# mightypirate1/DRL-Tetris

Hardware: AMD Instinct MI355X
Metric: env-steps/sec at 64k parallel 20x10 boards (higher is better)
Workload: dtype u32

## Files before the change

drl-tetris_amd/csrc/tetris_engine.h:

```cpp
#pragma once
#include "tetris_layout.h"
#include "tetris_tables.h"

#if defined(__clang__)
#define TE_UNROLL _Pragma("unroll")
#else
#define TE_UNROLL _Pragma("GCC unroll 8")
#endif

namespace te {

TE_HD int ctz32(uint32_t v) { return __builtin_ctz(v); }
TE_HD int clz32(uint32_t v) { return __builtin_clz(v); }
#if defined(__HIP_DEVICE_COMPILE__)
TE_HD uint32_t ld_stream(const uint32_t* p) { return __builtin_nontemporal_load(p); }
TE_HD void st_stream(uint32_t* p, uint32_t v) { __builtin_nontemporal_store(v, p); }
#else
TE_HD uint32_t ld_stream(const uint32_t* p) { return *p; }
TE_HD void st_stream(uint32_t* p, uint32_t v) { *p = v; }
#endif

#if defined(TE_PATH_COUNTERS) && !defined(__HIPCC__)
enum PathCounter { PC_KICK = 0, PC_KICK_2ND, PC_KICK_3RD, PC_KICK_FAILED, PC_KICK_DOWN, PC_DROP_EXACT, PC_RT_OFF_SPAWN,
                   PC_GARBAGE_ROW, PC_GARBAGE_LIFT2, PC_DEATH_GARBAGE, PC_DEATH_SPAWN, PC_TIMER_LOCK, PC_KEY_KICK, PC_KEY_KICK_FAILED,
                   PC_UNDO_SIMPLE, PC_UNDO_FULL, PC_UNDO_MISPREDICT, PC_NCOUNTERS };
extern unsigned long long te_path_count[PC_NCOUNTERS];
#define TE_COUNT(i) (te_path_count[i]++)
#else
#define TE_COUNT(i) do {} while (0)
#endif

enum MemMode : int { MEM_STREAM = 0, MEM_AGENT = 1, MEM_AFFINE = 2 };
#if defined(__HIP_DEVICE_COMPILE__)
TE_HD uint32_t ld_agent(const uint32_t* p) { return __hip_atomic_load(p, __ATOMIC_RELAXED, __HIP_MEMORY_SCOPE_AGENT); }
TE_HD void st_agent(uint32_t* p, uint32_t v) { __hip_atomic_store(p, v, __ATOMIC_RELAXED, __HIP_MEMORY_SCOPE_AGENT); }
#else
TE_HD uint32_t ld_agent(const uint32_t* p) { return *p; }
TE_HD void st_agent(uint32_t* p, uint32_t v) { *p = v; }
#endif
#if defined(__HIP_DEVICE_COMPILE__)
TE_HD __amdgpu_buffer_rsrc_t te_rsrc(const void* base) {
// ... 96 lines not shown
    const uint64_t* start;
    const double* combo_pow;
    uint32_t n_draws;
    uint32_t margin;
    int H;
    uint32_t floor_bits;
    bool tint;
    bool queue;
};

constexpr int ERR_FIFO = 1;
constexpr int ERR_STREAM = 2;

struct Raw8 { uint32_t lo, hi; };
struct Player {
    uint32_t col[NCOL];
    uint32_t tint[3][NCOL];
    int kind, rot, x, y, next;
    int dead, lock_armed, reward;
    int inc_count, combo_count, line_count, qlen;
    int q_overflow;
    int32_t time_ms, drop_delay, drop_time, speedup_time, lock_time;
    int32_t combo_start, combo_time, min_remaining;
    uint32_t combo_remaining;
    float incoming;
    uint32_t piece_draws, hole_draws;
    uint32_t pgroup;
    uint32_t lines_sent, lines_cleared, lines_blocked, max_combo, lines_seen, garbage_cleared;
    int32_t qcount[FIFO_CAP];
    int32_t qdelay[FIFO_CAP];
    int q_loaded;
    Raw8 pf_raw;
    int pf_ok;
};

struct ResetPrefetch { uint32_t seed16; uint64_t word; int ok; };

template <int P>
struct Game {
    Player pl[P];
    uint32_t seed16;
    int round_over, last_winner;
    uint32_t flags;
    uint32_t episode;
    uint32_t steps;
    uint32_t add_lines, add_sent;
    uint32_t status;
    uint32_t draw0, draw1;
};

template <class ROWS>
TE_HD void load_player_rows(const uint32_t* s, uint32_t o, const ROWS& rows, Player& q, bool tint, bool queue = true, int mem = MEM_STREAM,
                            bool errs = true) {
    for (int c = 0; c < NCOL; c++) q.col[c] = ldw_b(s, o, row_bytes(rows, W_COL0 + c), mem);
    if (tint)
        for (int k = 0; k < 3; k++)
            for (int c = 0; c < NCOL; c++) q.tint[k][c] = ldw_b(s, o, row_bytes(rows, W_TINT0 + 10 * k + c), mem);
    uint32_t w = ldw_b(s, o, row_bytes(rows, W_PIECE), mem);
    q.kind = w & 7; q.rot = (w >> 3) & 3; q.x = (int)((w >> 5) & 15) - 4; q.y = (w >> 9) & 31;
    q.next = (w >> 14) & 7; q.dead = (w >> 17) & 1; q.lock_armed = (w >> 18) & 1; q.reward = (w >> 19) & 255;
    w = ldw_b(s, o, row_bytes(rows, W_MISC), mem);
    q.inc_count = w & 255; q.combo_count = (w >> 8) & 255; q.line_count = (w >> 16) & 255;
    q.qlen = (w >> 24) & 15; q.q_overflow = (w >> 28) & 3;
    if (!queue) { q.inc_count = 0; q.qlen = 0; }
    if (!queue && !errs) q.q_overflow = 0;
    q.time_ms = (int32_t)ldw_b(s, o, row_bytes(rows, W_TIME), mem);
    w = ldw_b(s, o, row_bytes(rows, W_DROPCOMBO), mem);
    q.drop_delay = w & 0xFFFF; q.combo_remaining = w >> 16;
    q.drop_time = (int32_t)ldw_b(s, o, row_bytes(rows, W_DROP_TIME), mem);
    q.speedup_time = (int32_t)ldw_b(s, o, row_bytes(rows, W_SPEEDUP_TIME), mem);
    q.lock_time = (int32_t)ldw_b(s, o, row_bytes(rows, W_LOCK_TIME), mem);
    q.combo_start = (int32_t)ldw_b(s, o, row_bytes(rows, W_COMBO_START), mem);
    q.combo_time = (int32_t)ldw_b(s, o, row_bytes(rows, W_COMBO_TIME), mem);
    q.incoming = queue ? u2f(ldw_b(s, o, row_bytes(rows, W_INCOMING), mem)) : 0.0f;
    q.min_remaining = queue ? (int32_t)ldw_b(s, o, row_bytes(rows, W_MIN_REMAINING), mem) : 1000;
    q.piece_draws = ldw_b(s, o, row_bytes(rows, W_PIECE_DRAWS), mem);
    q.hole_draws = queue ? ldw_b(s, o, row_bytes(rows, W_HOLE_DRAWS), mem) : 0u;
    q.pgroup = ldw_b(s, o, row_bytes(rows, W_PIECE_GROUP), mem);
    w = ldw_b(s, o, row_bytes(rows, W_STATS0), mem); q.lines_sent = w & 0xFFFF; q.lines_cleared = w >> 16;
    w = ldw_b(s, o, row_bytes(rows, W_STATS1), mem); q.lines_blocked = w & 0xFFFF; q.max_combo = w >> 16;
    w = ldw_b(s, o, row_bytes(rows, W_STATS2), mem); q.lines_seen = w & 0xFFFF; q.garbage_cleared = w >> 16;
    q.q_loaded = queue && q.qlen > 0;
    q.pf_ok = 0; q.pf_raw.lo = 0; q.pf_raw.hi = 0;
    if (queue)
        for (int i = 0; i < FIFO_CAP; i++) { q.qcount[i] = 0; q.qdelay[i] = 0; }
    if (q.q_loaded) {
        for (int i = 0; i < FIFO_CAP / 2; i++) {
            uint32_t cw = ldw_b(s, o, row_bytes(rows, W_FIFO_COUNT0 + i), mem);
            q.qcount[2 * i] = (int16_t)(cw & 0xFFFF);
            q.qcount[2 * i + 1] = (int16_t)(cw >> 16);
        }
        for (int i = 0; i < FIFO_CAP; i++) q.qdelay[i] = (int32_t)ldw_b(s, o, row_bytes(rows, W_FIFO_DELAY0 + i), mem);
    }
}

TE_HD void load_player(const uint32_t* s, uint32_t o, size_t ws, Player& q, bool tint, bool queue = true, int mem = MEM_STREAM) {
    load_player_rows(s, o, RowStride{ws}, q, tint, queue, mem);
}

template <int P, class ROWS>
TE_HD void load_game_words_rows(const Ref& gr, const ROWS& rows, Game<P>& g, bool counters = false, int mem = MEM_STREAM) {
    uint32_t meta = ldw_b(gr.s, gr.o, row_bytes(rows, G_META), mem);
    g.seed16 = meta & 0xFFFFu;
    g.round_over = (meta >> 16) & 1;
    g.last_winner = (int)((meta >> 17) & 0xF) - 1;
    g.flags = (meta >> 21) & 7u;
    g.episode = ldw_b(gr.s, gr.o, row_bytes(rows, G_EPISODE), mem);
    g.steps = counters ? ldw_b(gr.s, gr.o, row_bytes(rows, G_STEPS), mem) : 0u;
    g.add_lines = 0; g.add_sent = 0;
    g.status = 0;
}

template <int P>
TE_HD void load_game_words(const Ref& gr, Game<P>& g, bool counters = false, int mem = MEM_STREAM) {
    load_game_words_rows<P>(gr, RowStride{gr.ws}, g, counters, mem);
}
// ... 27 lines not shown
    stw_b(s, o, row_bytes(rows, W_MISC), (uint32_t)(q.inc_count & 255) | ((uint32_t)(q.combo_count & 255) << 8) |
                             ((uint32_t)(q.line_count & 255) << 16) | ((uint32_t)q.qlen << 24) | ((uint32_t)q.q_overflow << 28), mem);
    stw_b(s, o, row_bytes(rows, W_TIME), (uint32_t)q.time_ms, mem);
    stw_b(s, o, row_bytes(rows, W_DROPCOMBO), ((uint32_t)q.drop_delay & 0xFFFF) | (q.combo_remaining << 16), mem);
    stw_b(s, o, row_bytes(rows, W_DROP_TIME), (uint32_t)q.drop_time, mem);
    stw_b(s, o, row_bytes(rows, W_SPEEDUP_TIME), (uint32_t)q.speedup_time, mem);
    stw_b(s, o, row_bytes(rows, W_LOCK_TIME), (uint32_t)q.lock_time, mem);
    stw_b(s, o, row_bytes(rows, W_COMBO_START), (uint32_t)q.combo_start, mem);
    stw_b(s, o, row_bytes(rows, W_COMBO_TIME), (uint32_t)q.combo_time, mem);
    if (queue) stw_b(s, o, row_bytes(rows, W_INCOMING), f2u(q.incoming), mem);
    stw_b(s, o, row_bytes(rows, W_MIN_REMAINING), (uint32_t)q.min_remaining, mem);
    stw_b(s, o, row_bytes(rows, W_PIECE_DRAWS), q.piece_draws, mem);
    if (queue) stw_b(s, o, row_bytes(rows, W_HOLE_DRAWS), q.hole_draws, mem);
    stw_b(s, o, row_bytes(rows, W_PIECE_GROUP), q.pgroup, mem);
    stw_b(s, o, row_bytes(rows, W_STATS0), (q.lines_sent & 0xFFFF) | (q.lines_cleared << 16), mem);
    stw_b(s, o, row_bytes(rows, W_STATS1), (q.lines_blocked & 0xFFFF) | (q.max_combo << 16), mem);
    stw_b(s, o, row_bytes(rows, W_STATS2), (q.lines_seen & 0xFFFF) | (q.garbage_cleared << 16), mem);
    if (queue && (q.q_loaded || q.qlen > 0)) {
        for (int i = 0; i < FIFO_CAP / 2; i++)
            stw_b(s, o, row_bytes(rows, W_FIFO_COUNT0 + i), ((uint32_t)q.qcount[2 * i] & 0xFFFF) | ((uint32_t)q.qcount[2 * i + 1] << 16), mem);
        for (int i = 0; i < FIFO_CAP; i++) stw_b(s, o, row_bytes(rows, W_FIFO_DELAY0 + i), (uint32_t)q.qdelay[i], mem);
    }
}

TE_HD void store_player(uint32_t* s, uint32_t o, size_t ws, const Player& q, bool tint, bool queue = true, int mem = MEM_STREAM) {
    store_player_rows(s, o, RowStride{ws}, q, tint, queue, mem);
}

template <int P, class ROWS>
TE_HD void store_game_words_rows(const Ref& gr, const ROWS& rows, const Game<P>& g, bool counters = false, int mem = MEM_STREAM) {
    stw_b(gr.s, gr.o, row_bytes(rows, G_META), g.seed16 | ((uint32_t)g.round_over << 16) | ((uint32_t)(g.last_winner + 1) << 17) | (g.flags << 21), mem);
    stw_b(gr.s, gr.o, row_bytes(rows, G_EPISODE), g.episode, mem);
    if (counters) stw_b(gr.s, gr.o, row_bytes(rows, G_STEPS), g.steps, mem);
    if (g.add_lines) add_word((uint32_t*)((char*)gr.s + row_bytes(rows, G_LINES) + gr.o), g.add_lines);
    if (g.add_sent) add_word((uint32_t*)((char*)gr.s + row_bytes(rows, G_SENT) + gr.o), g.add_sent);
}

template <int P>
TE_HD void store_game_words(const Ref& gr, const Game<P>& g, bool counters = false, int mem = MEM_STREAM) {
    store_game_words_rows<P>(gr, RowStride{gr.ws}, g, counters, mem);
}

template <int P, class ROWS, class GROWS>
TE_HD void store_game_rows(const Geo& geo_in, size_t slot, const ROWS& rows, const GROWS& grows, const Game<P>& g, bool tint = false, bool queue = true,
                           bool counters = false, int mem = MEM_STREAM) {
    Geo geo = geo_in;
    geo.P = P;
    store_game_words_rows<P>(game_ref(geo, slot), grows, g, counters, mem);
    TE_UNROLL
    for (int p = 0; p < P; p++) {
        const Ref r = board_ref(geo, p, slot);
        store_player_rows(r.s, r.o, rows, g.pl[p], tint, queue, mem);
    }
}
template <int P>
TE_HD void store_game(const Geo& geo_in, size_t slot, const Game<P>& g, bool tint = false, bool queue = true, bool counters = false, int mem = MEM_STREAM) {
    store_game_rows<P>(geo_in, slot, RowStride{(size_t)P * geo_in.stride}, RowStride{geo_in.stride}, g, tint, queue, counters, mem);
}


TE_HD uint32_t shape_of(const Ctx& cx, int kind, int rot) { return cx.shapes[(kind << 2) | rot]; }

TE_HD uint64_t band_window(const Ctx& cx, const Player& q, int y) {
    uint32_t lo = 0xFFu, hi = 0xFFFF0000u;
    for (int c = 0; c < 6; c++) lo |= ((uint32_t)((int32_t)(q.col[c] | cx.floor_bits) >> y) & 0xFu) << (4 * c + 8);
    for (int c = 6; c < NCOL; c++) hi |= ((uint32_t)((int32_t)(q.col[c] | cx.floor_bits) >> y) & 0xFu) << (4 * (c - 6));
    return ((uint64_t)hi << 32) | lo;
}
// ... 54 lines not shown
    const uint32_t lo = hi2 ? (hi1 ? 0u : w2) : (hi1 ? w1 : w0);
    const uint32_t hi = hi2 ? 0u : (hi1 ? w2 : w1);
#if defined(__HIP_DEVICE_COMPILE__)
    const uint32_t under = __builtin_amdgcn_alignbyte(hi, lo, xs & 3u);
#else
    const uint32_t under = (uint32_t)((((uint64_t)hi << 32) | lo) >> (8 * (xs & 3u)));
#endif
    const uint32_t sum = under + drop_word;
    const uint32_t b0 = sum & 0xFFu, b1 = (sum >> 8) & 0xFFu, b2 = (sum >> 16) & 0xFFu, b3 = sum >> 24;
    const uint32_t m01 = b0 < b1 ? b0 : b1, m23 = b2 < b3 ? b2 : b3;
    const uint32_t m = m01 < m23 ? m01 : m23;
    if (m - 0x40u > 0x3Eu) { TE_COUNT(PC_DROP_EXACT); return drop_distance(cx, q, shape); }
    return (int)(m - 0x40u);
}

TE_HD void stamp(const Ctx& cx, Player& q, uint32_t shape) {
    unsigned xs = (unsigned)(q.x + 2);
    if (xs > 12u) return;
    uint64_t placed = (uint64_t)(shape & 0xFFFFu) << (4 * xs);
    for (int c = 0; c < NCOL; c++) {
        const uint32_t cells = ((uint32_t)(placed >> (4 * c + 8)) & 0xFu) << q.y;
        q.col[c] |= cells;
        if (cx.tint)
            for (int k = 0; k < 3; k++) q.tint[k][c] = (q.tint[k][c] & ~cells) | (((q.kind >> k) & 1) ? cells : 0u);
    }
}

TE_HD int clear_rows(const Ctx& cx, Player& q) {
    uint32_t range = (~0u << q.y) & ~cx.floor_bits;
    int cleared = 0;
    for (;;) {
        uint32_t full = range;
        for (int c = 0; c < NCOL; c++) full &= q.col[c];
        if (!full) break;
        int r = 31 - clz32(full);
        uint32_t above = (1u << r) - 1u;
        uint32_t keep = ~((above << 1) | 1u);
        if (cx.tint) {
            uint32_t garbage = 0;
            for (int c = 0; c < NCOL; c++) garbage |= q.col[c] & q.tint[0][c] & q.tint[1][c] & q.tint[2][c];
            if ((garbage >> r) & 1u) q.garbage_cleared = (q.garbage_cleared + 1u) & 0xFFFFu;
            for (int k = 0; k < 3; k++)
                for (int c = 0; c < NCOL; c++) q.tint[k][c] = (q.tint[k][c] & keep) | ((q.tint[k][c] & above) << 1);
        }
        for (int c = 0; c < NCOL; c++) q.col[c] = (q.col[c] & keep) | ((q.col[c] & above) << 1);
        cleared++;
    }
    return cleared;
}

TE_HD uint32_t table_byte(const Ctx& cx, uint32_t seed16, uint32_t draw, uint32_t& status) {
    if (draw + cx.margin >= cx.n_draws) {
        status |= ST_NEED_EXTEND;
        if (draw >= cx.n_draws) { status |= ST_STREAM_EXHAUSTED; draw = cx.n_draws - 1; }
    }
    uint32_t chunk = draw / (uint32_t)CHUNK;
    uint32_t r = draw - mul24(chunk, (uint32_t)CHUNK);
    return cx.table[mul24((chunk << 16) + seed16, (uint32_t)CHUNK) + r];
}

TE_HD Raw8 table_group_raw(const Ctx& cx, uint32_t seed16, uint32_t draw, uint32_t& status) {
    if (draw + 8u + cx.margin >= cx.n_draws) {
        status |= ST_NEED_EXTEND;
        if (draw + 8u > cx.n_draws) { status |= ST_STREAM_EXHAUSTED; draw = cx.n_draws - 8u; }
    }
    uint32_t chunk = draw / (uint32_t)CHUNK;
    uint32_t r = draw - mul24(chunk, (uint32_t)CHUNK);
    const uint8_t* p = cx.table + (mul24((chunk << 16) + seed16, (uint32_t)CHUNK) + r);
    Raw8 v;
#if defined(__HIP_DEVICE_COMPILE__)
    const uint2 w = *reinterpret_cast<const uint2*>(p);
    v.lo = w.x; v.hi = w.y;
#else
    v.lo = 0; v.hi = 0;
    for (int k = 0; k < 4; k++) { v.lo |= (uint32_t)p[k] << (8 * k); v.hi |= (uint32_t)p[4 + k] << (8 * k); }
#endif
    return v;
}
TE_HD uint32_t pack_group(Raw8 v) {
    const uint32_t a = v.lo & 0x0F0F0F0Fu, b = v.hi & 0x0F0F0F0Fu;
    uint32_t lo = (a | (a >> 4)) & 0x00FF00FFu; lo = (lo | (lo >> 8)) & 0x0000FFFFu;
    uint32_t hi = (b | (b >> 4)) & 0x00FF00FFu; hi = (hi | (hi >> 8)) & 0x0000FFFFu;
    return lo | (hi << 16);
}

TE_HD void prefetch_next(const Ctx& cx, Player& q, uint32_t seed16, uint32_t& status) {
    q.pf_ok = 0;
    if ((q.piece_draws & 7u) == 7u) {
        q.pf_raw = table_group_raw(cx, seed16, q.piece_draws + 1u, status);
        q.pf_ok = 1;
    }
}

TE_HD void q_pop_front(Player& q) {
    for (int i = 0; i + 1 < FIFO_CAP; i++) { q.qcount[i] = q.qcount[i + 1]; q.qdelay[i] = q.qdelay[i + 1]; }
    q.qcount[FIFO_CAP - 1] = 0; q.qdelay[FIFO_CAP - 1] = 0;
    q.qlen--;
}

TE_HD void q_add(Player& q, int amount, int32_t t, uint32_t& status) {
    if (q.qlen >= FIFO_CAP) { q.q_overflow |= ERR_FIFO; status |= ST_FIFO_OVERFLOW; return; }
    for (int i = 0; i < FIFO_CAP; i++)
        if (i == q.qlen) { q.qcount[i] = (int16_t)amount; q.qdelay[i] = t + 1000; }
    q.qlen++;
}

TE_HD int q_block(Player& q, int amount, int32_t t, bool freeze) {
    if (q.qlen == 0) return amount;
    int32_t head_delay = q.qdelay[0];
    int blocked = 0;
    while (amount && q.qlen) {
        int take = imin(amount, (int)q.qcount[0]);
        if (take < 1) take = 1;
        q.qcount[0] -= take; amount -= take; blocked += take;
        if (q.qcount[0] == 0) q_pop_front(q);
    }
    q.lines_blocked = (q.lines_blocked + (uint32_t)blocked) & 0xFFFFu;
    if (q.qlen) {
        if (head_delay > q.qdelay[0]) q.qdelay[0] = head_delay;
        if (freeze) q.qdelay[0] = imin(q.qdelay[0] + 450, t + q.min_remaining + 450);
    } else
        q.min_remaining = 1000;
    return amount;
}
// ... 8 lines not shown
            q.min_remaining = q.qdelay[0] - t;
        } else
            q.min_remaining = 1000;
        return true;
    }
    q.min_remaining = imin(q.min_remaining, q.qdelay[0] - t);
    return false;
}

TE_HD int q_total(const Player& q) {
    uint32_t total = 0;
    for (int i = 0; i < FIFO_CAP; i++)
        if (i < q.qlen) total += (uint32_t)q.qcount[i];
    return (int)(total & 0xFFFFu);
}


TE_HD void combo_gain(Player& q, int32_t t, int amount) {
    if (q.combo_count == 0) { q.combo_start = t; q.combo_time = 0; }
    q.combo_count = (q.combo_count + 1) & 255;
    float line_time = 0.0f;
    for (int i = 0; i < amount; i++) {
        q.line_count = (q.line_count + 1) & 255;
        line_time = line_time + (float)(1000 / imax(1, q.line_count));
    }
    float add = (float)(800 / imax(1, q.combo_count)) + line_time;
    q.combo_time = (int32_t)((float)q.combo_time + add);
    if ((uint32_t)q.combo_count > q.max_combo) q.max_combo = (uint32_t)q.combo_count;
}

TE_HD int combo_expire(const Ctx& cx, Player& q, int32_t t) {
    int32_t left = q.combo_start + q.combo_time - t;
    q.combo_remaining = left < 0 ? 0u : ((uint32_t)left & 0xFFFFu);
    if (t > q.combo_start + q.combo_time && q.combo_count != 0) {
        float duration = 1.f + (float)t / 60000.f * 0.1f;
        double v = cx.combo_pow[q.combo_count] * (double)duration;
        int lines = (int)((uint32_t)(int64_t)v & 0xFFFFu);
        q.combo_count = 0;
        q.line_count = 0;
        return lines;
    }
    return 0;
}


TE_HD bool spawn_next(const Ctx& cx, Player& q, uint32_t seed16, uint32_t& status) {
    q.kind = q.next;
    q.rot = spawn_rot(q.kind);
    q.x = (NCOL - 4) / 2;
    q.y = 0;
    if (q.piece_draws + cx.margin >= cx.n_draws) {
        status |= ST_NEED_EXTEND;
        if (q.piece_draws >= cx.n_draws) status |= ST_STREAM_EXHAUSTED;
    }
    q.next = (int)((q.pgroup >> (4u * (q.piece_draws & 7u))) & 7u);
    q.piece_draws++;
    if ((q.piece_draws & 7u) == 0u) {
        q.pgroup = pack_group(q.pf_ok ? q.pf_raw : table_group_raw(cx, seed16, q.piece_draws, status));
        q.pf_ok = 0;
    }
    uint32_t shape = shape_of(cx, q.kind, q.rot);
    if (!fits_spawn_col(cx, q, shape, 0)) { stamp(cx, q, shape); TE_COUNT(PC_DEATH_SPAWN); return true; }
    return false;
}

TE_HD int score_clears(const Ctx& cx, Player& q, int cleared) {
    q.lines_cleared = (q.lines_cleared + (uint32_t)cleared) & 0xFFFFu;
    if (cleared == 0) { q.combo_time -= 200; return 0; }
    int amount = cx.queue ? q_block(q, cleared - 1, q.time_ms, true) : cleared - 1;
    q.lines_sent = (q.lines_sent + (uint32_t)amount) & 0xFFFFu;
    combo_gain(q, q.time_ms, cleared);
    return amount;
}

TE_HD void lock_piece(const Ctx& cx, Player& q) {
    uint32_t shape = shape_of(cx, q.kind, q.rot);
    q.y += drop_distance(cx, q, shape);
    stamp(cx, q, shape);
    q.drop_time = q.time_ms;
    q.lock_armed = 0;
}

TE_HD int settle(const Ctx& cx, Player& q, uint32_t seed16, uint32_t& status) {
    int sent = score_clears(cx, q, clear_rows(cx, q));
    if (spawn_next(cx, q, seed16, status)) return -1;
    return sent;
}

TE_HD bool soft_drop(const Ctx& cx, Player& q) {
    const uint32_t shape = shape_of(cx, q.kind, q.rot);
    if (q.x == (NCOL - 4) / 2 ? fits_spawn_col(cx, q, shape, q.y + 1) : fits_at(cx, q, shape, q.x, q.y + 1)) {
        q.y++;
        q.drop_time = q.time_ms;
        q.lock_armed = 0;
        return true;
    }
    if (!q.lock_armed) q.lock_time = q.time_ms + 400;
    q.lock_armed = 1;
    return false;
}

// ... 1 lines not shown
    if (t - q.speedup_time > 3000) {
        if (q.drop_delay > 200) q.drop_delay -= 10;
        else if (q.drop_delay > 100) q.drop_delay -= 5;
        else if (q.drop_delay > 50) q.drop_delay -= 2;
        else if (q.drop_delay > 10) q.drop_delay -= 1;
        q.speedup_time = t;
    }
    if (t - q.drop_time > q.drop_delay) { q.drop_time = t; return true; }
    return false;
}

TE_HD bool push_garbage(const Ctx& cx, Player& q, uint32_t seed16, uint32_t& status) {
    int hole = (int)(table_byte(cx, seed16, q.hole_draws, status) >> 4);
    q.hole_draws++;
    uint32_t bottom = 1u << (cx.H - 1);
    for (int c = 0; c < NCOL; c++) q.col[c] = (q.col[c] >> 1) | (c == hole ? 0u : bottom);
    if (cx.tint)
        for (int k = 0; k < 3; k++)
            for (int c = 0; c < NCOL; c++) q.tint[k][c] = (q.tint[k][c] >> 1) | (c == hole ? 0u : bottom);
    TE_COUNT(PC_GARBAGE_ROW);
    if (q.y > 0) q.y--;
    if (!fits_at(cx, q, shape_of(cx, q.kind, q.rot), q.x, q.y)) {
        if (q.y > 0) { q.y--; TE_COUNT(PC_GARBAGE_LIFT2); }
        else { TE_COUNT(PC_DEATH_GARBAGE); return true; }
    }
    return false;
}

TE_HD int tick(const Ctx& cx, Player& q, int ms, uint32_t seed16, uint32_t& status) {
    q.time_ms += ms;
    if (gravity_due(q, q.time_ms)) soft_drop(cx, q);
    int sent = 0;
    bool finished = false;
    if (q.lock_armed && q.time_ms > q.lock_time && !soft_drop(cx, q)) {
        TE_COUNT(PC_TIMER_LOCK);
        lock_piece(cx, q);
        sent = settle(cx, q, seed16, status);
        finished = true;
    }
    if (!finished) {
        if (cx.queue) {
            int whole = 0;
            while (q.incoming >= 1.0f) { whole++; q.incoming = q.incoming - 1.f; }
            if (whole) q_add(q, whole, q.time_ms, status);
        }
        sent = combo_expire(cx, q, q.time_ms);
        if (sent) {
            if (cx.queue) sent = q_block(q, sent, q.time_ms, false);
            q.lines_sent = (q.lines_sent + (uint32_t)sent) & 0xFFFFu;
        }
        if (cx.queue && q_release(q, q.time_ms))
            if (push_garbage(cx, q, seed16, status)) sent = -1;
    }
    return sent;
}

TE_HD void restart_player(const Ctx& cx, Player& q, uint32_t seed16, uint32_t& status, const ResetPrefetch* pf = nullptr) {
    for (int c = 0; c < NCOL; c++) q.col[c] = 0;
    if (cx.tint)
        for (int k = 0; k < 3; k++)
            for (int c = 0; c < NCOL; c++) q.tint[k][c] = 0;
    q.qlen = 0; q.q_overflow = 0; q.lines_blocked = 0; q.min_remaining = 1000;
    if (cx.queue)
        for (int i = 0; i < FIFO_CAP; i++) { q.qcount[i] = 0; q.qdelay[i] = 0; }
    q.combo_start = 0; q.combo_time = 0; q.max_combo = 0; q.combo_count = 0; q.line_count = 0;
    q.lines_sent = 0; q.lines_cleared = 0; q.garbage_cleared = 0;
    q.speedup_time = 0; q.drop_delay = 1000; q.drop_time = 0; q.lock_time = 0; q.lock_armed = 0;
    q.time_ms = 0; q.incoming = 0.0f; q.lines_seen = 0; q.dead = 0;
    (void)status;
    const uint64_t word = (pf && pf->ok && pf->seed16 == seed16) ? pf->word : cx.start[seed16];
    const uint32_t j = (uint32_t)word & 0xFFu, b0 = ((uint32_t)word >> 8) & 0xFFu, b1 = ((uint32_t)word >> 16) & 0xFFu;
    q.pgroup = (uint32_t)(word >> 32);
    q.kind = (int)(b0 & 7u);
    q.next = (int)(b1 & 7u);
    q.pf_ok = 0;
    q.rot = spawn_rot(q.kind);
    q.x = (NCOL - 4) / 2; q.y = 0;
    q.piece_draws = j + 2; q.hole_draws = 0;
}

template <int P>
TE_HD void reset_game(const Ctx& cx, Game<P>& g, uint32_t seed16, const ResetPrefetch* pf = nullptr) {
    g.round_over = 0;
    int winner = -1, alive = 0;
    TE_UNROLL
    for (int p = 0; p < P; p++)
        if (!g.pl[p].dead) { alive++; winner = p; }
    g.last_winner = winner;
    if (P == 1) g.last_winner = 0;
    if (alive > 1) g.last_winner = -1;
    g.seed16 = seed16 & 0xFFFFu;
    TE_UNROLL
    for (int p = 0; p < P; p++) restart_player(cx, g.pl[p], g.seed16, g.status, pf);
}

TE_HD void prefetch_reset(const Ctx& cx, uint32_t next_seed16, ResetPrefetch& pf) {
    pf.seed16 = next_seed16 & 0xFFFFu;
    pf.word = cx.start[pf.seed16];
    pf.ok = 1;
}

template <int P>
TE_HD void init_game(const Ctx& cx, Game<P>& g, uint32_t seed16) {
    TE_UNROLL
    for (int p = 0; p < P; p++) {
        Player& q = g.pl[p];
        q.reward = 0; q.inc_count = 0; q.combo_remaining = 0; q.dead = 0; q.next = 0; q.kind = 7; q.rot = 0;
        q.q_loaded = 1;
// ... 133 lines not shown
    uint32_t lo = 0xFFu, hi = 0xFFFF0000u;
    for (int c = 0; c < 6; c++) lo |= (r.v[c] & 0xFu) << (4 * c + 8);
    for (int c = 6; c < NCOL; c++) hi |= (r.v[c] & 0xFu) << (4 * (c - 6));
    return ((uint64_t)hi << 32) | lo;
}
TE_HD uint64_t band_one_down(uint64_t band, const RowsFrom& r) {
    uint32_t lo = (uint32_t)band, hi = (uint32_t)(band >> 32);
    lo = ((lo >> 1) & 0x77777777u) | 0xFFu;
    hi = ((hi >> 1) & 0x77777777u) | 0xFFFF0000u;
    for (int c = 0; c < 6; c++) lo |= (r.v[c] & 0x10u) << (4 * c + 7);
    hi |= (r.v[6] & 0x10u) >> 1;
    for (int c = 7; c < NCOL; c++) hi |= (r.v[c] & 0x10u) << (4 * (c - 6) - 1);
    return ((uint64_t)hi << 32) | lo;
}
TE_HD int drop_distance_rows(const Ctx& cx, const Player& q, const RowsFrom& r, uint32_t shape, uint32_t drop_word) {
    uint32_t d[NCOL];
    for (int c = 0; c < NCOL; c++) d[c] = (uint32_t)ctz32(r.v[c]);
    const uint32_t w0 = (d[0] << 16) | (d[1] << 24);
    const uint32_t w1 = d[2] | (d[3] << 8) | (d[4] << 16) | (d[5] << 24);
    const uint32_t w2 = d[6] | (d[7] << 8) | (d[8] << 16) | (d[9] << 24);
    const unsigned xs = (unsigned)(q.x + 2);
    const bool hi2 = (xs & 8u) != 0, hi1 = (xs & 4u) != 0;
    const uint32_t lo = hi2 ? (hi1 ? 0u : w2) : (hi1 ? w1 : w0);
    const uint32_t hi = hi2 ? 0u : (hi1 ? w2 : w1);
#if defined(__HIP_DEVICE_COMPILE__)
    const uint32_t under = __builtin_amdgcn_alignbyte(hi, lo, xs & 3u);
#else
    const uint32_t under = (uint32_t)((((uint64_t)hi << 32) | lo) >> (8 * (xs & 3u)));
#endif
    const uint32_t sum = under + drop_word;
    const uint32_t b0 = sum & 0xFFu, b1 = (sum >> 8) & 0xFFu, b2 = (sum >> 16) & 0xFFu, b3 = sum >> 24;
    const uint32_t m01 = b0 < b1 ? b0 : b1, m23 = b2 < b3 ? b2 : b3;
    const uint32_t m = m01 < m23 ? m01 : m23;
    if (m - 0x40u > 0x3Eu) { TE_COUNT(PC_DROP_EXACT); return drop_distance(cx, q, shape); }
    return (int)(m - 0x40u);
}

TE_HD void play_rt(const Ctx& cx, Player& q, int r, int t) {
    const Shapes4 sh = shapes_of_kind(cx, q.kind);
    const Shapes4 dw = drop_words_of_kind(cx, q.kind);
    if (q.y != 0 || q.x != (NCOL - 4) / 2) TE_COUNT(PC_RT_OFF_SPAWN);
    RowsFrom rows = rows_from(cx, q, q.y);
    uint64_t band = band_of_rows(rows);
    uint32_t win = band_win32(band, q.x);
    const bool fit1 = (((pick4(sh, q.rot + 1) & 0xFFFFu) << 8) & win) == 0;
    const bool fit2 = (((pick4(sh, q.rot + 2) & 0xFFFFu) << 8) & win) == 0;
    const bool fit3 = (((pick4(sh, q.rot + 3) & 0xFFFFu) << 8) & win) == 0;
    const bool easy = (r < 1 || fit1) && (r < 2 || fit2) && (r < 3 || fit3);
    if (easy) {
        q.rot = (q.rot + r) & 3;
    } else {
        int adv = fit1 ? (fit2 ? (fit3 ? 3 : 2) : 1) : 0;
        q.rot = (q.rot + adv) & 3;
        int left = r - adv;
        int kicks = 0;
        (void)kicks;
        while (left > 0) {
            const int nr = (q.rot + 1) & 3;
            const uint32_t s1 = pick4(sh, nr) & 0xFFFFu;
            const uint64_t b1 = band_one_down(band, rows);
            const uint32_t win1 = band_win32(b1, q.x);
            const uint32_t sA = s1, sB = s1 << 4, sC = s1 << 8, sD = s1 << 12, sE = s1 << 16;
            const bool k0 = (sC & win1) == 0, k1 = (sB & win) == 0, k2 = (sD & win) == 0;
            const bool k3 = (sB & win1) == 0, k4 = (sD & win1) == 0;
            const bool k5 = (sA & win) == 0, k6 = (sE & win) == 0;
            int dx = k6 ? 2 : 99, dy = 0;
            dx = k5 ? -2 : dx;
            if (k4) { dx = 1; dy = 1; }
            if (k3) { dx = -1; dy = 1; }
            if (k2) { dx = 1; dy = 0; }
            if (k1) { dx = -1; dy = 0; }
            if (k0) { dx = 0; dy = 1; }
            if (dx == 99) { TE_COUNT(PC_KICK_FAILED); break; }
            kicks++;
            TE_COUNT(kicks == 1 ? PC_KICK : (kicks == 2 ? PC_KICK_2ND : PC_KICK_3RD));
            if (dy) TE_COUNT(PC_KICK_DOWN);
            q.rot = nr; q.x += dx; q.y += dy;
            if (dy) {
                band = b1;
                for (int c = 0; c < NCOL; c++) rows.v[c] >>= 1;
            }
            left--;
// ... 254 lines not shown
    }
    return err != 0;
}

template <int P>
TE_HD int finish_game(const Ctx& cx, Game<P>& g, int ms) {
    if (g.round_over) return 1;
    bool stop = false;
    TE_UNROLL
    for (int p = 0; p < P; p++) {
        Player& q = g.pl[p];
        if (!stop && !q.dead) {
            const int sent = settle(cx, q, g.seed16, g.status);
            if (sent == -1) { q.dead = 1; stop = true; }
            else if (sent) share_lines<P>(g, p, sent);
        }
    }
    int alive = 0;
    TE_UNROLL
    for (int p = 0; p < P; p++) {
        Player& q = g.pl[p];
        if (!q.dead) {
            const int sent = tick(cx, q, ms, g.seed16, g.status);
            if (sent == -1) q.dead = 1;
            else {
                if (sent) share_lines<P>(g, p, sent);
                alive++;
                q.reward = (int)((q.lines_cleared - q.lines_seen) & 0xFFu);
                q.lines_seen = q.lines_cleared;
                q.inc_count = cx.queue ? (q_total(q) & 255) : 0;
            }
        }
    }
    if (confine_errors<P>(g)) { g.round_over = 1; return 1; }
    if ((P > 1 && alive < 2) || !alive) { g.round_over = 1; return 1; }
    return 0;
}

constexpr uint32_t XW_DIED = 1u << 16, XW_DEAD_NOW = 1u << 17, XW_RAN = 1u << 18, XW_ERR = 1u << 19;
constexpr uint32_t SPLIT_SIDE = 1u, SPLIT_OPP_DEAD = 2u, SPLIT_ON = 4u;
TE_HD int xw_sent(uint32_t w) { return (int)(w & 0xFFFFu); }

TE_HD uint32_t split_settle(const Ctx& cx, Game<1>& g) {
    Player& q = g.pl[0];
    if (g.round_over || q.dead) return 0u;
    int sent = settle(cx, q, g.seed16, g.status);
    if (g.status & ST_STREAM_EXHAUSTED) q.q_overflow |= ERR_STREAM;
    if (sent == -1) { q.dead = 1; return XW_RAN | XW_DIED; }
    return XW_RAN | (uint32_t)(sent & 0xFFFF);
}

TE_HD uint32_t split_tick(const Ctx& cx, Game<1>& g, int ms, int lines_in) {
    Player& q = g.pl[0];
    if (g.round_over) return (q.dead ? XW_DEAD_NOW : 0u) | (q.q_overflow ? XW_ERR : 0u);
    if (lines_in > 0) q.incoming = q.incoming + (float)lines_in / 1.0f;
    uint32_t w = 0;
    if (!q.dead) {
        int sent = tick(cx, q, ms, g.seed16, g.status);
        if (sent == -1) { q.dead = 1; w = XW_DIED; }
        else {
            w = (uint32_t)(sent & 0xFFFF);
            q.reward = (int)((q.lines_cleared - q.lines_seen) & 0xFFu);
            q.lines_seen = q.lines_cleared;
            q.inc_count = q_total(q) & 255;
        }
    }
    if (g.status & ST_STREAM_EXHAUSTED) q.q_overflow |= ERR_STREAM;
// ... 44 lines not shown
```

drl-tetris_amd/csrc/tetris_kernels.h:

```cpp
#pragma once
#include "../../include/tetris_hip.h"
#include "tetris_engine.h"

namespace te {

struct KArgs {
    uint32_t* state;
    uint32_t* gstate;
    uint32_t* status;
    const uint8_t* table;
    const uint64_t* start;
    const double* combo_pow;
    uint32_t n_draws, margin;
    int H;
    int n_games;
    int n_stride;
    int n_players;
    int nw;
    int n;
    const int32_t* idx;
    const uint8_t* keys;
    const uint8_t* lens;
    int max_keys;
    const uint8_t* rot;
// ... 17 lines not shown
    uint32_t xcd_slot;
    uint32_t* shadow;
    int split_side;
    const uint32_t* xw[4];
    uint32_t* xout;
    const uint8_t* next_player;
    uint8_t* obs_visual;
    uint8_t* obs_vector;
    uint8_t* obs_piece;
};

enum Mode { M_INIT, M_RESET, M_MAKE, M_FINISH, M_STEP_KEYS, M_STEP_RT, M_ROLLOUT, M_SPLIT_INIT, M_SPLIT_RESET,
            M_STEP_RT_AUTO,
            M_RESET_SCHED };

struct LaneCounters { unsigned long long steps, episodes, lines, sent; };

TE_HD size_t safe_slot(const int32_t* idx, int i, int n_games) {
    if (!idx) return (size_t)i;
    const uint32_t v = (uint32_t)idx[i];
    return (size_t)(v < (uint32_t)n_games ? v : (uint32_t)n_games - 1u);
}
TE_HD int safe_player_value(int v, int P) { return v < P ? v : P - 1; }
TE_HD int safe_player(const uint8_t* player, int i, int P) { return safe_player_value(player ? (int)player[i] : 0, P); }

TE_HD bool lane_active(const KArgs& a, int i) { return i < a.n && (!a.mask || a.mask[i] != 0); }

TE_HD Geo geo_of(const KArgs& a, uint32_t* state = nullptr) {
    Geo g = {state ? state : a.state, a.gstate, (size_t)a.n_games, a.n_players, a.nw, (size_t)a.n_stride};
    return g;
}

TE_HD void report_status(const KArgs& a, uint32_t st) {
    if (!st) return;
    volatile uint32_t* f = a.status;
    if (st & ST_NEED_EXTEND) f[F_EXTEND] = a.n_draws;
    if (st & ST_STREAM_EXHAUSTED) f[F_EXHAUSTED] = 1u;
    if (st & ST_FIFO_OVERFLOW) f[F_FIFO] = 1u;
    if (st & ST_BAD_ARGUMENT) f[F_BADARG] = 1u;
}

constexpr uint32_t CHAIN_ABANDONED = 0x80000000u;
constexpr uint32_t CHAIN_EPOCH_MAX = 0x7FFF0000u;
constexpr int CHAIN_STRIDE = 32;
constexpr int CHAIN_SLEEP = 1;
constexpr uint32_t CHAIN_SPIN_LIMIT = 1u << 22;

#if defined(__HIP_DEVICE_COMPILE__)
typedef __attribute__((address_space(1))) uint32_t te_gu32;
TE_HD void or_agent(uint32_t* p, uint32_t v) { (void)__hip_atomic_fetch_or(p, v, __ATOMIC_RELAXED, __HIP_MEMORY_SCOPE_AGENT); }
TE_HD void st_flag(uint32_t* p, uint32_t v) { __hip_atomic_store((te_gu32*)p, v, __ATOMIC_RELAXED, __HIP_MEMORY_SCOPE_SYSTEM); }
TE_HD uint32_t ld_flag(const uint32_t* p) { return __hip_atomic_load((const te_gu32*)p, __ATOMIC_RELAXED, __HIP_MEMORY_SCOPE_SYSTEM); }
TE_HD void st_xcd(uint32_t* p, uint32_t v) { __hip_atomic_store((te_gu32*)p, v, __ATOMIC_RELAXED, __HIP_MEMORY_SCOPE_WAVEFRONT); }
#else
TE_HD void or_agent(uint32_t* p, uint32_t v) { *p |= v; }
TE_HD void st_flag(uint32_t* p, uint32_t v) { *(volatile uint32_t*)p = v; }
TE_HD uint32_t ld_flag(const uint32_t* p) { return *(const volatile uint32_t*)p; }
TE_HD void st_xcd(uint32_t* p, uint32_t v) { *p = v; }
#endif

TE_HD uint32_t chain_poll(const KArgs& a, uint32_t wave) {
    const uint32_t want = a.epoch - 1u;
    const uint32_t* word = a.chain + (size_t)wave * CHAIN_STRIDE;
    uint32_t v = (uint32_t)wave_uniform(ld_agent(word));
    for (uint32_t polls = 1; v != want && !(v & CHAIN_ABANDONED) && polls < a.chain_spin_limit; polls++) {
        if ((polls & 255u) == 0 && wave_uniform(ld_flag(a.status + F_PLACE)) != 0) break;
#if defined(__HIP_DEVICE_COMPILE__)
// ... 64 lines not shown
        Player& q = g.pl[p];
        int len = a.lens[(size_t)p * a.n + i];
        if (q.dead) len = 0;
        for (int k = 0; k < len; k++) press_key(cx, q, a.keys[((size_t)k * P + p) * a.n + i]);
    }
}

template <int P>
TE_HD void make_rt(const Ctx& cx, Game<P>& g, int player, int r, int t) {
    if (g.round_over) return;
    TE_UNROLL
    for (int p = 0; p < P; p++)
        if (p == player && !g.pl[p].dead) play_rt(cx, g.pl[p], r, t);
}

TE_HD void policy_draw(const KArgs& a, uint32_t slot, unsigned long long step, uint32_t& w0, uint32_t& w1) {
    uint32_t w[4];
    philox4x32_10(a.policy_seed, a.game_offset + slot, (uint32_t)step, (uint32_t)(step >> 32), w);
    w0 = w[0]; w1 = w[1];
}

template <int P, int MODE, bool TINT = false, int MEM = MEM_STREAM>
TE_HD void game_load(const KArgs& a, int i, Game<P>& g) {
    const size_t slot = a.idx ? (size_t)a.idx[i] : (size_t)i;
    if (MODE != M_INIT && MODE != M_SPLIT_INIT)
        load_game<P>(geo_of(a), slot, g, TINT, P > 1 || MODE == M_SPLIT_RESET, MODE == M_ROLLOUT, MEM);
    if (MODE == M_ROLLOUT) policy_draw(a, (uint32_t)slot, a.first_step, g.draw0, g.draw1);
    if (MODE == M_STEP_RT || MODE == M_STEP_RT_AUTO) { g.draw0 = a.rot[i]; g.draw1 = (uint32_t)a.trans[i] | ((a.player ? (uint32_t)a.player[i] : 0u) << 8); }
}

template <int P>
TE_HD void rollout_step(const Ctx& cx, const KArgs& a, size_t slot, unsigned long long step, Game<P>& g, LaneCounters& cnt) {
    TE_UNROLL
    for (int p = 0; p < P; p++) prefetch_next(cx, g.pl[p], g.seed16, g.status);
    ResetPrefetch rpf;
    prefetch_reset(cx, episode_seed(a.game_offset + (uint32_t)slot, g.episode + 1), rpf);
    int r = (int)(g.draw0 & 3u), t = (int)(g.draw1 % 10u);
    int player = P > 1 ? (int)(step % (unsigned long long)P) : 0;
    uint32_t sent_before = 0;
    TE_UNROLL
    for (int p = 0; p < P; p++) sent_before += g.pl[p].lines_sent;
    make_rt<P>(cx, g, player, r, t);
    int done = finish_game<P>(cx, g, a.ms);
    cnt.steps++;
    g.steps++;
    uint32_t sent_after = 0;
    TE_UNROLL
    for (int p = 0; p < P; p++) {
        sent_after += g.pl[p].lines_sent;
        if (!g.pl[p].dead) { cnt.lines += (unsigned)g.pl[p].reward; g.add_lines += (unsigned)g.pl[p].reward; }
    }
    cnt.sent += (sent_after - sent_before) & 0xFFFFu;
    g.add_sent += (sent_after - sent_before) & 0xFFFFu;
    if (done) {
        cnt.episodes++;
        g.episode++;
        reset_game<P>(cx, g, episode_seed(a.game_offset + (uint32_t)slot, g.episode), &rpf);
    }
}

template <int P, int MODE, bool TINT = false, int MEM = MEM_STREAM>
TE_HD void game_run(const KArgs& a, int i, const uint32_t* shapes, Game<P>& g, LaneCounters& cnt) {
    const size_t slot = a.idx ? (size_t)a.idx[i] : (size_t)i;
    Ctx cx = make_ctx(a, shapes, TINT, P > 1 || MODE == M_SPLIT_INIT || MODE == M_SPLIT_RESET);
    if (MODE == M_INIT) init_game<P>(cx, g, (uint32_t)(a.seeds ? (uint16_t)a.seeds[i] : 0));
    if (MODE == M_SPLIT_INIT) {
        init_game<P>(cx, g, (uint32_t)(a.seeds ? (uint16_t)a.seeds[i] : 0));
// ... 455 lines not shown
```

Measured before the change: 22.45 billion.

## Prefetch next spawn shape and mark rare branches with expect hints

```diff
diff --git a/drl-tetris_amd/csrc/tetris_engine.h b/drl-tetris_amd/csrc/tetris_engine.h
--- a/drl-tetris_amd/csrc/tetris_engine.h
+++ b/drl-tetris_amd/csrc/tetris_engine.h
@@ -7,6 +7,7 @@
 #else
 #define TE_UNROLL _Pragma("GCC unroll 8")
 #endif
+#define TE_RARE(c) __builtin_expect(!!(c), 0)
 
 namespace te {
 
@@ -169,6 +170,8 @@
     int q_loaded;
     Raw8 pf_raw;
     int pf_ok;
+    uint32_t ns_shape;
+    int ns_ok;
 };
 
 struct ResetPrefetch { uint32_t seed16; uint64_t word; int ok; };
@@ -219,6 +222,7 @@
     w = ldw_b(s, o, row_bytes(rows, W_STATS2), mem); q.lines_seen = w & 0xFFFF; q.garbage_cleared = w >> 16;
     q.q_loaded = queue && q.qlen > 0;
     q.pf_ok = 0; q.pf_raw.lo = 0; q.pf_raw.hi = 0;
+    q.ns_ok = 0; q.ns_shape = 0;
     if (queue)
         for (int i = 0; i < FIFO_CAP; i++) { q.qcount[i] = 0; q.qdelay[i] = 0; }
     if (q.q_loaded) {
@@ -312,8 +316,8 @@
     stw_b(gr.s, gr.o, row_bytes(rows, G_META), g.seed16 | ((uint32_t)g.round_over << 16) | ((uint32_t)(g.last_winner + 1) << 17) | (g.flags << 21), mem);
     stw_b(gr.s, gr.o, row_bytes(rows, G_EPISODE), g.episode, mem);
     if (counters) stw_b(gr.s, gr.o, row_bytes(rows, G_STEPS), g.steps, mem);
-    if (g.add_lines) add_word((uint32_t*)((char*)gr.s + row_bytes(rows, G_LINES) + gr.o), g.add_lines);
-    if (g.add_sent) add_word((uint32_t*)((char*)gr.s + row_bytes(rows, G_SENT) + gr.o), g.add_sent);
+    if (TE_RARE(g.add_lines != 0)) add_word((uint32_t*)((char*)gr.s + row_bytes(rows, G_LINES) + gr.o), g.add_lines);
+    if (TE_RARE(g.add_sent != 0)) add_word((uint32_t*)((char*)gr.s + row_bytes(rows, G_SENT) + gr.o), g.add_sent);
 }
 
 template <int P>
@@ -434,7 +438,7 @@
     for (;;) {
         uint32_t full = range;
         for (int c = 0; c < NCOL; c++) full &= q.col[c];
-        if (!full) break;
+        if (!TE_RARE(full != 0)) break;
         int r = 31 - clz32(full);
         uint32_t above = (1u << r) - 1u;
         uint32_t keep = ~((above << 1) | 1u);
@@ -462,7 +466,7 @@
 }
 
 TE_HD Raw8 table_group_raw(const Ctx& cx, uint32_t seed16, uint32_t draw, uint32_t& status) {
-    if (draw + 8u + cx.margin >= cx.n_draws) {
+    if (TE_RARE(draw + 8u + cx.margin >= cx.n_draws)) {
         status |= ST_NEED_EXTEND;
         if (draw + 8u > cx.n_draws) { status |= ST_STREAM_EXHAUSTED; draw = cx.n_draws - 8u; }
     }
@@ -479,6 +483,11 @@
 #endif
     return v;
 }
+TE_HD void wait_vector_loads() {
+#if defined(__HIP_DEVICE_COMPILE__)
+    __builtin_amdgcn_s_waitcnt(0x0F70);
+#endif
+}
 TE_HD uint32_t pack_group(Raw8 v) {
     const uint32_t a = v.lo & 0x0F0F0F0Fu, b = v.hi & 0x0F0F0F0Fu;
     uint32_t lo = (a | (a >> 4)) & 0x00FF00FFu; lo = (lo | (lo >> 8)) & 0x0000FFFFu;
@@ -492,6 +501,11 @@
         q.pf_raw = table_group_raw(cx, seed16, q.piece_draws + 1u, status);
         q.pf_ok = 1;
     }
+}
+
+TE_HD void prefetch_spawn_shape(const Ctx& cx, Player& q) {
+    q.ns_shape = shape_of(cx, q.next, spawn_rot(q.next));
+    q.ns_ok = 1;
 }
 
 TE_HD void q_pop_front(Player& q) {
@@ -566,7 +580,7 @@
 TE_HD int combo_expire(const Ctx& cx, Player& q, int32_t t) {
     int32_t left = q.combo_start + q.combo_time - t;
     q.combo_remaining = left < 0 ? 0u : ((uint32_t)left & 0xFFFFu);
-    if (t > q.combo_start + q.combo_time && q.combo_count != 0) {
+    if (TE_RARE(t > q.combo_start + q.combo_time && q.combo_count != 0)) {
         float duration = 1.f + (float)t / 60000.f * 0.1f;
         double v = cx.combo_pow[q.combo_count] * (double)duration;
         int lines = (int)((uint32_t)(int64_t)v & 0xFFFFu);
@@ -583,24 +597,31 @@
     q.rot = spawn_rot(q.kind);
     q.x = (NCOL - 4) / 2;
     q.y = 0;
-    if (q.piece_draws + cx.margin >= cx.n_draws) {
+    if (TE_RARE(q.piece_draws + cx.margin >= cx.n_draws)) {
         status |= ST_NEED_EXTEND;
         if (q.piece_draws >= cx.n_draws) status |= ST_STREAM_EXHAUSTED;
     }
+    const uint32_t shape = q.ns_ok ? q.ns_shape : shape_of(cx, q.kind, q.rot);
     q.next = (int)((q.pgroup >> (4u * (q.piece_draws & 7u))) & 7u);
     q.piece_draws++;
     if ((q.piece_draws & 7u) == 0u) {
-        q.pgroup = pack_group(q.pf_ok ? q.pf_raw : table_group_raw(cx, seed16, q.piece_draws, status));
+        Raw8 raw = q.pf_raw;
+        if (TE_RARE(!q.pf_ok)) {
+            raw = table_group_raw(cx, seed16, q.piece_draws, status);
+            wait_vector_loads();
+        }
+        q.pgroup = pack_group(raw);
         q.pf_ok = 0;
     }
-    uint32_t shape = shape_of(cx, q.kind, q.rot);
-    if (!fits_spawn_col(cx, q, shape, 0)) { stamp(cx, q, shape); TE_COUNT(PC_DEATH_SPAWN); return true; }
+    const bool fits = fits_spawn_col(cx, q, shape, 0);
+    if (q.ns_ok) q.ns_shape = shape_of(cx, q.next, spawn_rot(q.next));
+    if (!fits) { stamp(cx, q, shape); TE_COUNT(PC_DEATH_SPAWN); return true; }
     return false;
 }
 
 TE_HD int score_clears(const Ctx& cx, Player& q, int cleared) {
     q.lines_cleared = (q.lines_cleared + (uint32_t)cleared) & 0xFFFFu;
-    if (cleared == 0) { q.combo_time -= 200; return 0; }
+    if (!TE_RARE(cleared != 0)) { q.combo_time -= 200; return 0; }
     int amount = cx.queue ? q_block(q, cleared - 1, q.time_ms, true) : cleared - 1;
     q.lines_sent = (q.lines_sent + (uint32_t)amount) & 0xFFFFu;
     combo_gain(q, q.time_ms, cleared);
@@ -668,7 +689,7 @@
     if (gravity_due(q, q.time_ms)) soft_drop(cx, q);
     int sent = 0;
     bool finished = false;
-    if (q.lock_armed && q.time_ms > q.lock_time && !soft_drop(cx, q)) {
+    if (TE_RARE(q.lock_armed && q.time_ms > q.lock_time) && !soft_drop(cx, q)) {
         TE_COUNT(PC_TIMER_LOCK);
         lock_piece(cx, q);
         sent = settle(cx, q, seed16, status);
@@ -681,7 +702,7 @@
             if (whole) q_add(q, whole, q.time_ms, status);
         }
         sent = combo_expire(cx, q, q.time_ms);
-        if (sent) {
+        if (TE_RARE(sent != 0)) {
             if (cx.queue) sent = q_block(q, sent, q.time_ms, false);
             q.lines_sent = (q.lines_sent + (uint32_t)sent) & 0xFFFFu;
         }
@@ -704,12 +725,16 @@
     q.speedup_time = 0; q.drop_delay = 1000; q.drop_time = 0; q.lock_time = 0; q.lock_armed = 0;
     q.time_ms = 0; q.incoming = 0.0f; q.lines_seen = 0; q.dead = 0;
     (void)status;
-    const uint64_t word = (pf && pf->ok && pf->seed16 == seed16) ? pf->word : cx.start[seed16];
+    uint64_t word = pf ? pf->word : 0;
+    if (TE_RARE(!(pf && pf->ok && pf->seed16 == seed16))) {
+        word = cx.start[seed16];
+        wait_vector_loads();
+    }
     const uint32_t j = (uint32_t)word & 0xFFu, b0 = ((uint32_t)word >> 8) & 0xFFu, b1 = ((uint32_t)word >> 16) & 0xFFu;
     q.pgroup = (uint32_t)(word >> 32);
     q.kind = (int)(b0 & 7u);
     q.next = (int)(b1 & 7u);
-    q.pf_ok = 0;
+    q.pf_ok = 0; q.ns_ok = 0;
     q.rot = spawn_rot(q.kind);
     q.x = (NCOL - 4) / 2; q.y = 0;
     q.piece_draws = j + 2; q.hole_draws = 0;
@@ -909,7 +934,7 @@
     const uint32_t b0 = sum & 0xFFu, b1 = (sum >> 8) & 0xFFu, b2 = (sum >> 16) & 0xFFu, b3 = sum >> 24;
     const uint32_t m01 = b0 < b1 ? b0 : b1, m23 = b2 < b3 ? b2 : b3;
     const uint32_t m = m01 < m23 ? m01 : m23;
-    if (m - 0x40u > 0x3Eu) { TE_COUNT(PC_DROP_EXACT); return drop_distance(cx, q, shape); }
+    if (TE_RARE(m - 0x40u > 0x3Eu)) { TE_COUNT(PC_DROP_EXACT); return drop_distance(cx, q, shape); }
     return (int)(m - 0x40u);
 }
 
@@ -924,7 +949,7 @@
     const bool fit2 = (((pick4(sh, q.rot + 2) & 0xFFFFu) << 8) & win) == 0;
     const bool fit3 = (((pick4(sh, q.rot + 3) & 0xFFFFu) << 8) & win) == 0;
     const bool easy = (r < 1 || fit1) && (r < 2 || fit2) && (r < 3 || fit3);
-    if (easy) {
+    if (!TE_RARE(!easy)) {
         q.rot = (q.rot + r) & 3;
     } else {
         int adv = fit1 ? (fit2 ? (fit3 ? 3 : 2) : 1) : 0;
@@ -1245,7 +1270,7 @@
             }
         }
     }
-    if (confine_errors<P>(g)) { g.round_over = 1; return 1; }
+    if (TE_RARE(confine_errors<P>(g))) { g.round_over = 1; return 1; }
     if ((P > 1 && alive < 2) || !alive) { g.round_over = 1; return 1; }
     return 0;
 }
diff --git a/drl-tetris_amd/csrc/tetris_kernels.h b/drl-tetris_amd/csrc/tetris_kernels.h
--- a/drl-tetris_amd/csrc/tetris_kernels.h
+++ b/drl-tetris_amd/csrc/tetris_kernels.h
@@ -73,7 +73,7 @@
 }
 
 TE_HD void report_status(const KArgs& a, uint32_t st) {
-    if (!st) return;
+    if (!TE_RARE(st != 0)) return;
     volatile uint32_t* f = a.status;
     if (st & ST_NEED_EXTEND) f[F_EXTEND] = a.n_draws;
     if (st & ST_STREAM_EXHAUSTED) f[F_EXHAUSTED] = 1u;
@@ -204,7 +204,10 @@
 template <int P>
 TE_HD void rollout_step(const Ctx& cx, const KArgs& a, size_t slot, unsigned long long step, Game<P>& g, LaneCounters& cnt) {
     TE_UNROLL
-    for (int p = 0; p < P; p++) prefetch_next(cx, g.pl[p], g.seed16, g.status);
+    for (int p = 0; p < P; p++) {
+        prefetch_next(cx, g.pl[p], g.seed16, g.status);
+        prefetch_spawn_shape(cx, g.pl[p]);
+    }
     ResetPrefetch rpf;
     prefetch_reset(cx, episode_seed(a.game_offset + (uint32_t)slot, g.episode + 1), rpf);
     int r = (int)(g.draw0 & 3u), t = (int)(g.draw1 % 10u);
```

Result: no change. 22.63 billion, median of 6 (+0.8%).
